# garymm/starflate

Hardware: AMD Instinct MI355X
Metric: compress MiB/s + ratio vs zlib -6, 1 GiB synthetic; 1/2/4/8 GPU (higher is better)
Workload: dtype u8; 1 GPU; 1 GiB synthetic enwik-like text per GPU (gen_text_torch seed 3); effort=default, block_bytes=524288, deflate_block_bytes=32768, window_bytes=32768, container=raw, parallelism=shard1

## Files before the change

### starflate_amd/csrc/sf_kernels.hip

```cpp
#include "sf_device.h"

#include <stdlib.h>

namespace sf {

__device__ __forceinline__ uint32_t len_symbol(uint32_t l3, uint32_t& ebits, uint32_t& eval) {
  if (l3 == 255) { ebits = 0; eval = 0; return 285; }
  if (l3 < 8) { ebits = 0; eval = 0; return 257 + l3; }
  const uint32_t e = (31 - __builtin_clz(l3)) - 2;
  ebits = e;
  eval = l3 & ((1u << e) - 1);
  return 257 + 4 * e + 4 + ((l3 >> e) & 3);
}
__device__ __forceinline__ uint32_t dist_symbol(uint32_t d1, uint32_t& ebits, uint32_t& eval) {
  if (d1 < 4) { ebits = 0; eval = 0; return d1; }
  const uint32_t hb = 31 - __builtin_clz(d1);
  const uint32_t e = hb - 1;
  ebits = e;
  eval = d1 & ((1u << e) - 1);
  return 2 * hb + ((d1 >> e) & 1);
}
__device__ __forceinline__ uint32_t dist_symbol_of(uint32_t d1) {
  const uint32_t x = d1 > 2u ? d1 : 2u;
  const uint32_t hb = 31 - __builtin_clz(x);
// ... 1416 lines not shown
    if (lane < 29) hist[(uint64_t)chunk * kHistStride + 257 + lane] = S.freq[257 + lane];
  }

  stamp();
  if (MODE == 1 && strategy == 0) {
    uint32_t fixb = 0, extra = 0, tot = 0;
    for (uint32_t s0 = lane; s0 < 286; s0 += 64) tot += S.freq[s0];
    tot = wave_sum(tot);
    const uint32_t ltot = est_log2(tot);
    uint32_t ent = 0;
    for (uint32_t s0 = lane; s0 < 286; s0 += 64) {
      const uint32_t f = S.freq[s0];
      if (f) ent += f * (ltot - est_log2(f));
      fixb += f * fixed_ll_len(s0);
      if (s0 >= 257) extra += f * len_extra_of_sym(s0 - 257);
    }
    const uint32_t g = lane < 30 ? S.freq[kHistD + lane] : 0u;
    const uint32_t nmat = wave_sum(g);
    if (g) ent += g * (est_log2(nmat) - est_log2(g));
    if (lane < 30) extra += g * dist_extra_of_sym(lane);
    const uint32_t extra_all = wave_sum(extra);
    const uint32_t est_bits = (wave_sum(ent) >> 8) + extra_all + kEstHeaderBits;
    const uint32_t fixbits = 3 + wave_sum(fixb) + extra_all + 5 * nmat;
    const uint32_t est_b = fin ? (est_bits + 7) / 8 : (est_bits + 3 + 7) / 8 + 4;
    const uint32_t fix_b = fin ? (fixbits + 7) / 8 : (fixbits + 3 + 7) / 8 + 4;
    const uint32_t sto_b = n_raw + kStoredExtra;
    if (fix_b >= sto_b && est_b + kStoreMargin >= sto_b) {
      ChunkCodes& C0 = codes[chunk];
      for (uint32_t s0 = lane; s0 < 320; s0 += 64) C0.lens[s0] = 0;
      if (lane == 0) {
        C0.header[0] = fin ? 1u : 0u;
        ChunkPlan P;
        P.btype = 0;
        P.out_bytes = sto_b;
        P.header_bits = 3;
        P.body_bits = 0;
        plan[chunk] = P;
        T->done = 1;
      }
      return;
    }
  }
  if constexpr (MODE == 1) {
    const uint32_t m_ll = sort_symbols<5>(S, S.freq, 286, S.lens, lane);
    if (m_ll >= 2)
      for (uint32_t k = lane; k < m_ll; k += 64) {
        const uint32_t key = S.key[k];
        T->key_ll[k] = key;
        T->wt_ll[k] = (uint16_t)(key >> 9);
      }
    __syncthreads();
    const uint32_t m_d = sort_symbols<1>(S, S.freq + kHistD, 30, S.lens + 288, lane);
    if (m_d >= 2 && lane < m_d) {
      const uint32_t key = S.key[lane];
      T->key_d[lane] = key;
      T->wt_d[lane] = (uint16_t)(key >> 9);
    }
    if (lane == 0) { T->done = 0; T->m_ll = m_ll; T->m_d = m_d; }
    return;
  } else {
    const uint32_t m_ll = T->m_ll, m_d = T->m_d;
    if (m_ll < 2) {
      sort_symbols<5>(S, S.freq, 286, S.lens, lane);
    } else {
      if (lane < 16) S.cnt[lane] = 0;
      for (uint32_t k = lane; k < m_ll; k += 64) S.key[k] = T->key_ll[k];
      for (uint32_t v = lane; v < 2 * m_ll - 2; v += 64) S.parent[v] = T->parent_ll[v];
      __syncthreads();
      finish_lengths(S, m_ll, 15, S.lens, lane);
    }
    stamp();
    if (m_d < 2) {
      sort_symbols<1>(S, S.freq + kHistD, 30, S.lens + 288, lane);
    } else {
      if (lane < 16) S.cnt[lane] = 0;
      if (lane < m_d) S.key[lane] = T->key_d[lane];
      if (lane < 2 * m_d - 2) S.parent[lane] = T->parent_d[lane];
      __syncthreads();
      finish_lengths(S, m_d, 15, S.lens + 288, lane);
    }
    stamp();
  }

  uint32_t dyn = 0, fix = 0, extra = 0, nmatch = 0;
  for (uint32_t s = lane; s < 286; s += 64) {
    const uint32_t f = S.freq[s];
    dyn += f * S.lens[s];
    fix += f * fixed_ll_len(s);
    if (s >= 257) extra += f * len_extra_of_sym(s - 257);
  }
  if (lane < 30) {
    const uint32_t f = S.freq[kHistD + lane];
    dyn += f * S.lens[288 + lane];
    extra += f * dist_extra_of_sym(lane);
    nmatch += f;
  }
  dyn = wave_sum(dyn);
  fix = wave_sum(fix);
  extra = wave_sum(extra);
  nmatch = wave_sum(nmatch);
  const uint32_t dyn_body = dyn + extra;
  const uint32_t fix_body = fix + extra + 5 * nmatch;

  if (lane < 32) S.clfreq[lane] = 0;
  for (uint32_t k = lane; k < kHeaderWords; k += 64) s_header[k] = 0;
  __syncthreads();
  uint32_t hlit, hdist;
  {
    const uint64_t m4 = __ballot(256 + lane < 286 && S.lens[256 + lane] != 0);
    hlit = 256 + 64 - (uint32_t)__builtin_clzll(m4);
    const uint64_t md = __ballot(lane < 30 && S.lens[288 + lane] != 0);
    hdist = md ? 64 - (uint32_t)__builtin_clzll(md) : 1u;
  }
  const uint32_t nl = rle_parallel(S, S.lens, hlit, 0, lane);
  const uint32_t nd = rle_parallel(S, S.lens + 288, hdist, nl, lane);
  const uint32_t nitems = nl + nd;
  __syncthreads();
  stamp();
  build_lengths(S, S.clfreq, 19, 7, S.cl_lens, lane);
  canonical_codes(S.cl_lens, 19, S.cl_code, lane);
  __syncthreads();
  stamp();
  {
    const uint64_t mc = __ballot(lane < 19 && S.cl_lens[c_cl_order[lane < 19 ? lane : 0]] != 0);
    uint32_t hclen = mc ? 64 - (uint32_t)__builtin_clzll(mc) : 4u;
    hclen = hclen < 4 ? 4u : hclen;
    if (lane == 0)
      or_bits(s_header, 0, (uint64_t)((fin ? 1u : 0u) | (2u << 1) | ((hlit - 257) << 3) | ((hdist - 1) << 8) | ((hclen - 4) << 13)));
    if (lane < hclen) or_bits(s_header, 17 + 3 * lane, (uint64_t)S.cl_lens[c_cl_order[lane]]);
    uint32_t bitbase = 17 + 3 * hclen;
#pragma unroll
    for (uint32_t g = 0; g < 5; ++g) {
      if (g * 64 >= nitems) break;
      const uint32_t k = g * 64 + lane;
      uint32_t nb = 0;
      uint64_t v = 0;
      if (k < nitems) {
        const uint32_t sy = S.rle_sym[k];
        const uint32_t c = S.cl_code[sy];
        const uint32_t cl = c >> 16;
        const uint32_t eb = sy == 16 ? 2u : sy == 17 ? 3u : sy == 18 ? 7u : 0u;
        v = (uint64_t)(c & 0xFFFF) | ((uint64_t)S.rle_ext[k] << cl);
        nb = cl + eb;
      }
      const uint32_t incl = wave_incl_add(nb);
      if (nb) or_bits(s_header, bitbase + incl - nb, v);
      bitbase += (uint32_t)__builtin_amdgcn_readlane((int)incl, 63);
    }
    if (lane == 0) S.cnt[0] = bitbase;
  }
  __syncthreads();

  stamp();
  const uint32_t dyn_hbits = S.cnt[0];
  const uint32_t dyn_bits = dyn_hbits + dyn_body;
  const uint32_t fix_bits = 3 + fix_body;
  const uint32_t dyn_bytes = fin ? (dyn_bits + 7) / 8 : (dyn_bits + 3 + 7) / 8 + 4;
  const uint32_t fix_bytes = fin ? (fix_bits + 7) / 8 : (fix_bits + 3 + 7) / 8 + 4;
  const uint32_t sto_bytes = n_raw + kStoredExtra;
  uint32_t bt;
  if (strategy == 1) bt = 0;
  else if (strategy == 2) bt = 1;
  else if (strategy == 3) bt = 2;
  else {
    bt = 0;
    uint32_t best = sto_bytes;
    if (fix_bytes < best) { bt = 1; best = fix_bytes; }
    if (dyn_bytes < best) { bt = 2; best = dyn_bytes; }
  }

  ChunkCodes& C = codes[chunk];
  for (uint32_t s = lane; s < 320; s += 64) C.lens[s] = S.lens[s];
  __syncthreads();
  if (bt == 1) {
    for (uint32_t s = lane; s < 320; s += 64) S.lens[s] = s < 288 ? (uint8_t)fixed_ll_len(s) : (uint8_t)5;
    if (lane == 0) s_header[0] = (fin ? 1u : 0u) | (1u << 1);
    __syncthreads();
  } else if (bt == 0) {
    if (lane == 0) s_header[0] = fin ? 1u : 0u;
    __syncthreads();
  }
  canonical_codes(S.lens, 288, C.lcode, lane);
  canonical_codes(S.lens + 288, 32, C.dcode, lane);
  const uint32_t hbits = bt == 2 ? dyn_hbits : 3;
  for (uint32_t k = lane; k < (hbits + 31) / 32; k += 64) C.header[k] = s_header[k];
  if (lane == 0) {
    ChunkPlan P;
    P.btype = bt;
    P.out_bytes = bt == 0 ? sto_bytes : bt == 1 ? fix_bytes : dyn_bytes;
    P.header_bits = hbits;
    P.body_bits = bt == 1 ? fix_body : dyn_body;
    plan[chunk] = P;
  }
  stamp();
}

#define SF_PLAN_KERNEL(NAME, MODE)                                                                                          \
  __global__ __launch_bounds__(64) void NAME(uint64_t n_total, uint32_t nchunks, uint32_t* __restrict__ hist,                 \
                                             const uint32_t* __restrict__ ntok, ChunkPlan* __restrict__ plan,                 \
                                             ChunkCodes* __restrict__ codes, uint32_t strategy, uint32_t final_stream,        \
                                             uint64_t* __restrict__ stamps, PlanTree* __restrict__ ptree,                     \
                                             const BatchChunk* __restrict__ bchunks) {                                        \
    plan_chunk<MODE>(n_total, nchunks, hist, ntok, plan, codes, strategy, final_stream, stamps, ptree, bchunks);              \
  }
SF_PLAN_KERNEL(k_plan_sort, 1)
SF_PLAN_KERNEL(k_plan_finish, 2)
#undef SF_PLAN_KERNEL

constexpr uint32_t KM_ROW = 289;
static_assert(2 * KM_ROW >= 576 && (KM_ROW & 1) == 1 && 64 * KM_ROW * 4 <= 80 * 1024, "k_plan_merge: two waves per CU");
__global__ __launch_bounds__(64) void k_plan_merge(uint32_t nchunks, PlanTree* __restrict__ ptree) {
  __shared__ uint32_t s_rows[64 * KM_ROW];
  const uint32_t lane = threadIdx.x;
  const uint32_t chunk = blockIdx.x * 64 + lane;
  if (chunk >= nchunks) return;
  PlanTree* const T = ptree + chunk;
  if (T->done) return;
  uint16_t* const w = reinterpret_cast<uint16_t*>(s_rows + lane * KM_ROW);
  uint32_t* const w32 = s_rows + lane * KM_ROW;
#pragma unroll 1
  for (uint32_t tree = 0; tree < 2; ++tree) {
    const uint32_t m = tree ? T->m_d : T->m_ll;
    if (m < 2) continue;
    const uint32_t* const wt32 = reinterpret_cast<const uint32_t*>(tree ? T->wt_d : T->wt_ll);
    uint16_t* const parent = tree ? T->parent_d : T->parent_ll;
    for (uint32_t k = 0; k < (m + 1) / 2; ++k) w32[k] = wt32[k];
    merge_two_queue_lane(m, [&](uint32_t k) -> uint32_t { return w[k]; }, [&](uint32_t k, uint32_t v) { w[k] = (uint16_t)v; },
                         [&](uint32_t x, uint32_t k) { parent[x] = (uint16_t)k; });
  }
}

constexpr uint32_t K3_THREADS = 1024;
constexpr uint32_t K3_TILES = kBatchChunks / K3_THREADS;
static_assert(kBatchChunks % K3_THREADS == 0 && K3_TILES == 32 && K3_THREADS / 64 == 16, "k_scan: 32 tiles, a DPP row per tile's wave totals");
static_assert((uint64_t)kBatchChunks * (kChunk + kChunk / 8 + 656) < (1ull << 32), "a batch's bytes fit 32 bits");
template <bool BATCH>
__global__ __launch_bounds__(K3_THREADS) void k_scan(uint32_t nchunks, const ChunkPlan* __restrict__ plan,
                                                     uint64_t base, uint32_t carry, uint64_t* __restrict__ offsets,
                                                     uint64_t* __restrict__ total, BatchItem* __restrict__ bitems,
                                                     uint32_t nitems) {
  __shared__ uint32_t s_wt[K3_TILES][16];
  __shared__ uint32_t s_tile[K3_TILES + 1];
  const uint64_t hdr = base;
  if constexpr (BATCH) base = 0;
  else if (carry) base = *total;
  const uint32_t t = threadIdx.x, lane = t & 63, wave = t >> 6;
  uint32_t v[K3_TILES], ex[K3_TILES];
#pragma unroll
  for (uint32_t k = 0; k < K3_TILES; ++k) {
    const uint32_t c = k * K3_THREADS + t;
    v[k] = c < nchunks ? plan[c].out_bytes : 0u;
  }
#pragma unroll
  for (uint32_t k = 0; k < K3_TILES; ++k) {
    const uint32_t incl = wave_incl_add(v[k]);
    ex[k] = incl - v[k];
    if (lane == 63) s_wt[k][wave] = incl;
  }
  __syncthreads();
  if (t < K3_TILES * 16) {
    const uint32_t x = s_wt[t >> 4][t & 15];
    uint32_t r = x;
    r += dpp_from<0x111, 0xF>(r);
    r += dpp_from<0x112, 0xF>(r);
    r += dpp_from<0x114, 0xF>(r);
    r += dpp_from<0x118, 0xF>(r);
    s_wt[t >> 4][t & 15] = r - x;
    if ((t & 15) == 15) s_tile[t >> 4] = r;
  }
  __syncthreads();
  if (wave == 0) {
    const uint32_t x = lane < K3_TILES ? s_tile[lane] : 0u;
    const uint32_t r = wave_incl_add(x);
    if (lane < K3_TILES) s_tile[lane] = r - x;
    if (lane == K3_TILES - 1) s_tile[K3_TILES] = r;
  }
  __syncthreads();
#pragma unroll
  for (uint32_t k = 0; k < K3_TILES; ++k) {
    const uint32_t c = k * K3_THREADS + t;
    if (c < nchunks) offsets[c] = base + s_tile[k] + s_wt[k][wave] + ex[k];
  }
  if (t == 0) {
    const uint64_t all = base + s_tile[K3_TILES];
    if constexpr (!BATCH) *total = all;
    offsets[nchunks] = all;
  }
  if constexpr (BATCH) {
    __syncthreads();
    for (uint32_t i = t; i < nitems; i += K3_THREADS) {
      BatchItem& I = bitems[i];
      const uint64_t g0 = offsets[I.chunk0], g1 = offsets[I.chunk0 + I.nchunks];
      const uint64_t start = I.carry ? total[I.out] : hdr;
      I.shift = start - g0;
      total[I.out] = start + (g1 - g0);
    }
  }
}

constexpr uint32_t K4_THREADS = 512;
constexpr uint32_t K4_WAVES = K4_THREADS / 64;
constexpr uint32_t K4_IPT = 8;
constexpr uint32_t K4_STAGE_FORCED = 9392;
constexpr uint32_t K4_STAGE_AUTO = 8200;
static_assert(4 * K4_STAGE_FORCED >= 3 + kChunk + kChunk / 8 + 640 + 16 + 8, "k_emit: the stage holds the largest chunk");
static_assert(4 * K4_STAGE_AUTO >= 3 + kChunk + kStoredExtra - 1 + 16 + 8, "k_emit: the small stage holds the largest chunk "
              "plan_chunk codes under strategy 0");
static_assert(K4_STAGE_FORCED % 4 == 0 && K4_STAGE_AUTO % 4 == 0, "the stage is zeroed in 16-byte steps");
template <uint32_t STAGE_WORDS>
struct EmitLds {
  alignas(16) uint32_t stage[STAGE_WORDS];
  uint32_t lcode[288];
  uint32_t dcode[32];
  uint32_t tab[1024];
  uint32_t wtot[2][K4_WAVES];
  uint32_t rtok[kSubRegions];
};
template <uint32_t STAGE_WORDS>
constexpr uint32_t k4_waves_per_simd() { return STAGE_WORDS == K4_STAGE_AUTO ? 8 : 6; }
static_assert(k4_waves_per_simd<K4_STAGE_AUTO>() / 2 * sizeof(EmitLds<K4_STAGE_AUTO>) <= 160 * 1024, "k_emit: four workgroups per CU");
static_assert(k4_waves_per_simd<K4_STAGE_FORCED>() / 2 * sizeof(EmitLds<K4_STAGE_FORCED>) <= 160 * 1024, "k_emit: three workgroups per CU");

typedef uint16_t u16x2 __attribute__((ext_vector_type(2)));
typedef int16_t s16x2 __attribute__((ext_vector_type(2)));

__device__ __forceinline__ void literal_bits(uint32_t byte, const uint32_t* lcode, uint64_t& value, uint32_t& nb) {
  const uint32_t lc = lcode[byte];
  value = lc & 0xFFFF;
  nb = lc >> 16;
}
__device__ __forceinline__ uint32_t lenlut_entry(uint32_t l3, const uint32_t* lcode) {
  uint32_t le, lv;
  const uint32_t lc = lcode[len_symbol(l3, le, lv)];
  const uint32_t p = lc >> 16;
  return (lc & 0xFFFFu) | (lv << p) | ((p + le) << 24);
}
__device__ __forceinline__ void match_bits(uint32_t l3, uint32_t d1, const uint32_t* lenlut, const uint32_t* dcode,
                                           uint64_t& value, uint32_t& nb) {
  uint32_t de, dv;
  const uint32_t ds = dist_symbol(d1, de, dv);
  const uint32_t le = lenlut[l3], dc = dcode[ds];
  uint32_t p = le >> 24;
  uint64_t v = le & 0xFFFFFFu;
  v |= (uint64_t)(dc & 0xFFFF) << p;
  p += dc >> 16;
  v |= (uint64_t)dv << p;
  p += de;
  value = v;
  nb = p;
}

template <bool BATCH, uint32_t STAGE_WORDS>
__global__ __launch_bounds__(K4_THREADS, k4_waves_per_simd<STAGE_WORDS>()) void k_emit(const uint8_t* __restrict__ src, uint64_t n_total,
                                                     uint32_t , uint16_t* items,
                                                     const uint32_t* __restrict__ nitems_in,
                                                     const uint32_t* __restrict__ ntok_in,
                                                     const ChunkPlan* __restrict__ plan,
                                                     const ChunkCodes* __restrict__ codes,
                                                     const uint64_t* __restrict__ offsets,
                                                     const uint32_t* __restrict__ rtok,
                                                     uint32_t* __restrict__ subidx,
                                                     uint8_t* __restrict__ dst_all,
                                                     const BatchChunk* __restrict__ bchunks,
                                                     const BatchItem* __restrict__ bitems) {
  __shared__ EmitLds<STAGE_WORDS> L;
  uint32_t(&s_stage)[STAGE_WORDS] = L.stage;
  uint32_t(&s_lcode)[288] = L.lcode;
  uint32_t(&s_dcode)[32] = L.dcode;
  uint32_t(&s_tab)[1024] = L.tab;
  uint32_t(&s_wtot)[2][K4_WAVES] = L.wtot;
  uint32_t(&s_rtok)[kSubRegions] = L.rtok;
  static_assert(K4_THREADS == 512, "one table entry per thread and kind");
  constexpr uint32_t kTabLit = 512, kTabLen = 768, kTabDistN = 510;

  const uint32_t t = threadIdx.x, lane = t & 63;
  const uint32_t wave = (uint32_t)__builtin_amdgcn_readfirstlane((int)(t >> 6));
  const uint32_t chunk = blockIdx.x;
  const ChunkPlan P = plan[chunk];
  const uint8_t* csrc;
  uint8_t* dst;
  uint64_t off = offsets[chunk];
  uint32_t n_raw;
  if constexpr (BATCH) {
    const BatchChunk B = bchunks[chunk];
    const BatchItem& I = bitems[B.item >> 1];
    csrc = B.src;
    n_raw = B.n_raw;
    dst = I.dst;
    off += I.shift;
  } else {
    const uint64_t cbase = (uint64_t)chunk * kChunk;
    csrc = src + cbase;
    n_raw = (uint32_t)((n_total - cbase) < (uint64_t)kChunk ? (n_total - cbase) : kChunk);
    dst = dst_all;
  }
  const ChunkCodes& C = codes[chunk];
  uint32_t pre_code = t < 288 ? C.lcode[t] : (t < 320 ? C.dcode[t - 288] : 0u);
  uint32_t pre_rtok = t < kSubRegions ? rtok[(uint64_t)chunk * kSubRegions + t] : 0u;
  const uint32_t pre_ntok = ntok_in[chunk], pre_nit = nitems_in[chunk];
  asm volatile("" : "+v"(pre_code), "+v"(pre_rtok));

  uint32_t* const sub = subidx + (uint64_t)chunk * 2 * kSubRegions;
  if (P.btype == 0) {
    if (t < 2 * kSubRegions) sub[t] = 0;
    uint8_t* o = dst + off;
    if (t == 0) {
      o[0] = (uint8_t)(C.header[0] & 1u);
      o[1] = (uint8_t)(n_raw & 0xFF);
      o[2] = (uint8_t)(n_raw >> 8);
      o[3] = (uint8_t)(~n_raw & 0xFF);
      o[4] = (uint8_t)((~n_raw >> 8) & 0xFF);
    }
    uint8_t* d = o + 5;
    const uint8_t* sp = csrc;
    if (n_raw >= 64) {
      const uint32_t head16 = (uint32_t)((16 - ((uintptr_t)d & 15)) & 15);
      if (t < head16) d[t] = sp[t];
      const uint32_t sft = head16 & 15u, wsel = sft >> 2, bs = sft & 3u;
      const uint32_t nvec = (n_raw - head16) / 16 - (sft ? 1u : 0u);
      const uint4* s4 = reinterpret_cast<const uint4*>(sp);
      uint4* d4 = reinterpret_cast<uint4*>(d + head16);
      for (uint32_t k = t; k < nvec; k += K4_THREADS) {
        const uint4 A = s4[k + (head16 >> 4)], B = sft ? s4[k + (head16 >> 4) + 1] : make_uint4(0, 0, 0, 0);
        uint4 r;
        if (wsel == 0) {
          r.x = __builtin_amdgcn_alignbyte(A.y, A.x, bs); r.y = __builtin_amdgcn_alignbyte(A.z, A.y, bs);
          r.z = __builtin_amdgcn_alignbyte(A.w, A.z, bs); r.w = __builtin_amdgcn_alignbyte(B.x, A.w, bs);
        } else if (wsel == 1) {
          r.x = __builtin_amdgcn_alignbyte(A.z, A.y, bs); r.y = __builtin_amdgcn_alignbyte(A.w, A.z, bs);
          r.z = __builtin_amdgcn_alignbyte(B.x, A.w, bs); r.w = __builtin_amdgcn_alignbyte(B.y, B.x, bs);
        } else if (wsel == 2) {
          r.x = __builtin_amdgcn_alignbyte(A.w, A.z, bs); r.y = __builtin_amdgcn_alignbyte(B.x, A.w, bs);
          r.z = __builtin_amdgcn_alignbyte(B.y, B.x, bs); r.w = __builtin_amdgcn_alignbyte(B.z, B.y, bs);
        } else {
          r.x = __builtin_amdgcn_alignbyte(B.x, A.w, bs); r.y = __builtin_amdgcn_alignbyte(B.y, B.x, bs);
          r.z = __builtin_amdgcn_alignbyte(B.z, B.y, bs); r.w = __builtin_amdgcn_alignbyte(B.w, B.z, bs);
        }
        d4[k] = r;
      }
      const uint32_t done16 = head16 + 16 * nvec;
      if (t < n_raw - done16) d[done16 + t] = sp[done16 + t];
      return;
    }
    const uint32_t head = (uint32_t)((4 - ((uintptr_t)d & 3)) & 3);
    const uint32_t h = head < n_raw ? head : n_raw;
    if (t < h) d[t] = sp[t];
    const uint32_t nd = (n_raw - h) / 4;
    uint32_t* d32 = reinterpret_cast<uint32_t*>(d + h);
    const uint32_t* s32 = reinterpret_cast<const uint32_t*>(sp);
    const uint32_t full_src_words = n_raw / 4;
    for (uint32_t k = t; k < nd; k += K4_THREADS) {
      const uint32_t ob = h + 4 * k;
      const uint32_t w = ob >> 2;
      uint32_t lo = s32[w], hi = 0;
      if ((ob & 3) != 0) {
        if (w + 1 < full_src_words) hi = s32[w + 1];
        else
          for (uint32_t b = 0; b < 4 && 4 * (w + 1) + b < n_raw; ++b) hi |= (uint32_t)sp[4 * (w + 1) + b] << (8 * b);
      }
      d32[k] = __builtin_amdgcn_alignbyte(hi, lo, ob & 3);
    }
    const uint32_t done = h + 4 * nd;
    if (t < n_raw - done) d[done + t] = sp[done + t];
    return;
  }

  const uint32_t sh = (uint32_t)(off & 3);
  const uint32_t nwords = (sh + P.out_bytes + 3) / 4;
  {
    uint4* z = reinterpret_cast<uint4*>(s_stage);
    for (uint32_t k = t; k < (nwords + 2 + 3) / 4 && k < STAGE_WORDS / 4; k += K4_THREADS) z[k] = make_uint4(0, 0, 0, 0);
  }
  if (t < 288) s_lcode[t] = pre_code;
  else if (t < 320) s_dcode[t - 288] = pre_code;
  if (t < kSubRegions) {
    s_rtok[t] = pre_rtok;
    sub[2 * t + 1] = pre_rtok;
  }
  __syncthreads();
  if (t < 256) {
    const uint32_t le = lenlut_entry(t, s_lcode);
    s_tab[kTabLen + t] = (le & 0xFFFFFu) | (le >> 24) * (1u << 20 | 1u << 27);
    s_tab[kTabLit + t] = (pre_code & 0xFFFFu) | (pre_code >> 16) * (1u << 20 | 1u << 27);
  }
  if (t < kTabDistN) {
    const uint32_t sym = dist_symbol_of(t < 256 ? t : (t - 254) << 7);
    const uint32_t dc = s_dcode[sym];
    s_tab[t] = (dc & 0xFFFFu) | ((dc >> 16) << 20) | (((dc >> 16) + dist_extra_of_sym(sym)) << 27);
  } else {
    s_tab[t] = 0;
  }
  {
    uint8_t* sb = reinterpret_cast<uint8_t*>(s_stage) + sh;
    const uint8_t* hb = reinterpret_cast<const uint8_t*>(C.header);
    const uint32_t hbytes = (P.header_bits + 7) / 8;
    for (uint32_t k = t; k < hbytes; k += K4_THREADS) sb[k] = hb[k];
  }
  __syncthreads();

  const uint32_t ntok = pre_ntok;
  const uint32_t nit = pre_nit & ~kItemsSkipped;
  const uint16_t* it = items + (uint64_t)chunk * kChunk;
  if (pre_nit & kItemsSkipped) {
    uint16_t* const wr = items + (uint64_t)chunk * kChunk;
    for (uint32_t pos = t; pos < nit; pos += K4_THREADS) {
      const uint32_t b = csrc[pos];
      wr[pos] = (uint16_t)(kItemTok | ((pos & (kSubBytes - 1)) == 0 ? (b | kItemRegion | ((pos / kSubBytes) << kItemRegionShift)) : b));
    }
    __threadfence_block();
    __syncthreads();
  }
  uint32_t running = 8 * sh + P.header_bits;
  uint32_t buf = 0;
  uint4 q_next = make_uint4(0, 0, 0, 0);
  if (nit) q_next = *reinterpret_cast<const uint4*>(it + t * K4_IPT);
  for (uint32_t b0 = 0; b0 < nit; b0 += K4_THREADS * K4_IPT, buf ^= 1) {
    const uint32_t i0 = b0 + t * K4_IPT;
    const uint4 q = q_next;
    const bool full = b0 + K4_THREADS * K4_IPT <= nit;
    if (b0 + K4_THREADS * K4_IPT < nit) q_next = *reinterpret_cast<const uint4*>(it + i0 + K4_THREADS * K4_IPT);
    const uint32_t qd[K4_IPT / 2] = {q.x, q.y, q.z, q.w};
    uint32_t val[K4_IPT], nb[K4_IPT], mine = 0;
    uint32_t ent[K4_IPT];
#pragma unroll
    for (uint32_t j = 0; j < K4_IPT / 2; ++j) {
      static_assert(kItemHead == 0x100 && kTabLen == kTabLit + 0x100 && kTabLit == 0x200, "a token's low nine bits are its table index");
      static_assert(kItemTok == 0x8000, "bit 15 tells a token's first item from a distance");
      const u16x2 w = __builtin_bit_cast(u16x2, qd[j]);
      const uint32_t itok = (qd[j] & 0x01FF01FFu) | (kTabLit * 0x10001u);
      const u16x2 idist = __builtin_elementwise_min(w, (u16x2)(w >> (uint16_t)7) + (uint16_t)254);
      uint32_t tok = __builtin_bit_cast(uint32_t, __builtin_bit_cast(s16x2, w) >> (int16_t)15);
      asm volatile("" : "+v"(tok));
      const uint32_t idx = (tok & itok) | (~tok & __builtin_bit_cast(uint32_t, idist));
      const uint32_t by = __builtin_bit_cast(uint32_t, (u16x2)(__builtin_bit_cast(u16x2, idx) << (uint16_t)2));
      ent[2 * j] = *reinterpret_cast<const uint32_t*>(reinterpret_cast<const uint8_t*>(s_tab) + (by & 0xFFFFu));
      ent[2 * j + 1] = *reinterpret_cast<const uint32_t*>(reinterpret_cast<const uint8_t*>(s_tab) + (by >> 16));
    }
    asm volatile("" : "+v"(ent[0]), "+v"(ent[1]), "+v"(ent[2]), "+v"(ent[3]), "+v"(ent[4]), "+v"(ent[5]), "+v"(ent[6]), "+v"(ent[7]));
    auto both = [](uint32_t w) { return w & (w << 1) & 0x80008000u; };
    auto sbit = [](uint32_t k) { return (k & 1) ? 15 + k : k; };
    uint32_t starts = (both(q.x) >> 15) | (both(q.y) >> 13) | (both(q.z) >> 11) | (both(q.w) >> 9);
    if (!full) {
      uint32_t left = nit - i0;
      left = i0 < nit ? left : 0u;
#pragma unroll
      for (uint32_t k = 0; k < K4_IPT; ++k) {
        ent[k] = k < left ? ent[k] : 0u;
        starts &= k < left ? ~0u : ~(1u << sbit(k));
      }
    }
    const uint32_t s0 = starts ? (uint32_t)__builtin_ctz(starts) : 32u;
    const bool walk = __ballot((starts & (starts - 1)) != 0) != 0;
    uint32_t off0 = 0;
#pragma unroll
    for (uint32_t k = 0; k < K4_IPT; ++k) {
      const uint32_t en = ent[k];
      const uint32_t dl = en >> 20, n = en >> 27;
      val[k] = (__builtin_amdgcn_ubfe(qd[k / 2], 16 * (k & 1), (n - dl) & 31u) << (dl & 31u)) | (en & 0xFFFFFu);
      nb[k] = n;
      asm volatile("" : "+v"(val[k]), "+v"(nb[k]));
      off0 = s0 == sbit(k) ? mine : off0;
      mine += nb[k];
    }
    uint32_t region0;
    {
      const uint32_t j = (s0 >> 1) & 3u;
      const uint32_t w = j == 0 ? q.x : j == 1 ? q.y : j == 2 ? q.z : q.w;
      region0 = (w >> ((s0 & 16u) + kItemRegionShift)) & 31u;
    }
    const uint32_t incl = wave_incl_add(mine);
    if (lane == 63) s_wtot[buf][wave] = incl;
    __syncthreads();
    uint32_t pre = 0, all = 0;
#pragma unroll
    for (uint32_t w = 0; w < K4_WAVES; ++w) {
      const uint32_t v = s_wtot[buf][w];
      if (w < wave) pre += v;
      all += v;
    }
    const uint32_t pos = running + pre + incl - mine;
    if (walk) {
      const uint4 r = *reinterpret_cast<const uint4*>(it + i0);
      const uint32_t rd[K4_IPT / 2] = {r.x, r.y, r.z, r.w};
      uint32_t pk = pos;
#pragma unroll
      for (uint32_t k = 0; k < K4_IPT; ++k) {
        const uint32_t e = (rd[k / 2] >> (16 * (k & 1))) & 0xFFFFu;
        if ((e & (kItemTok | kItemRegion)) == (kItemTok | kItemRegion) && i0 + k < nit)
          sub[2 * ((e >> kItemRegionShift) & 31u)] = pk - 8 * sh;
        pk += nb[k];
      }
    } else if (starts) {
      sub[2 * region0] = pos + off0 - 8 * sh;
    }
    uint32_t wi = pos >> 5, ab = pos & 31;
    uint64_t acc = 0;
    auto put = [&](uint32_t v32, uint32_t n) {
      acc |= (uint64_t)v32 << ab;
      ab += n;
      if (ab >= 32) {
        atomicOr(&s_stage[wi++], (uint32_t)acc);
        acc >>= 32;
        ab -= 32;
      }
    };
#pragma unroll
    for (uint32_t k = 0; k < K4_IPT; ++k) put(val[k], nb[k]);
    if (ab) atomicOr(&s_stage[wi], (uint32_t)acc);
    running += all;
  }
  __syncthreads();
  if (t < kSubRegions && s_rtok[t] >= ntok) sub[2 * t] = running - 8 * sh;
  if (t == 0) {
    const uint32_t eob = s_lcode[256];
    or_bits(s_stage, running, eob & 0xFFFF);
    const uint32_t endbit = running + (eob >> 16);
    if (!(C.header[0] & 1u)) {
      const uint32_t byte = (endbit + 3 + 7) / 8;
      or_bits(s_stage, 8 * (byte + 2), 0xFFFFull);
    }
  }
  __syncthreads();

  uint8_t* gbase = dst + (off - sh);
  uint32_t* g32 = reinterpret_cast<uint32_t*>(gbase);
  const uint32_t lo_b = sh, hi_b = sh + P.out_bytes;
  for (uint32_t w = t; w < nwords; w += K4_THREADS) {
    const uint32_t v = s_stage[w];
    if (4 * w >= lo_b && 4 * w + 4 <= hi_b) {
      g32[w] = v;
    } else {
#pragma unroll
      for (uint32_t b = 0; b < 4; ++b) {
        const uint32_t idx = 4 * w + b;
        if (idx >= lo_b && idx < hi_b) gbase[idx] = (uint8_t)(v >> (8 * b));
      }
    }
  }
}

hipError_t init_kernels() { return hipSuccess; }

hipError_t launch_lz77(const uint8_t* src, uint64_t n, uint32_t nchunks, const Workspace& ws,
                       const Options& opt, hipStream_t s, const BatchTables* bt) {
  if (opt.strip_bytes == 0 || opt.strip_bytes % kChunk || opt.strip_bytes > kMaxStrip) return hipErrorInvalidValue;
  if (opt.fast_skip == 2 && opt.strategy != 0) return hipErrorInvalidValue;
  const uint32_t per = opt.strip_bytes / kChunk;
  const uint32_t nstrips = bt ? bt->nstrips : (nchunks + per - 1) / per;
  const BatchStrip* strips = bt ? bt->strips : nullptr;
  const auto launch = [&](auto kernel, uint64_t* stamps) {
    hipLaunchKernelGGL(kernel, dim3(nstrips), dim3(K1_THREADS), 0, s, src, n, opt.strip_bytes, ws.items, ws.nitems, ws.ntok,
                       ws.hist, ws.rtok, opt.lazy, opt.fast_skip, stamps, opt.chain_depth, strips);
  };
#define SF_K1(D2, NR, S2, LG, CH, RC)                                                                                     \
  (ws.stamps && !bt ? launch(k_lz77<true, D2, NR, S2, LG, CH, RC>, ws.stamps)                                          \
   : !bt ? launch(k_lz77<false, D2, NR, S2, LG, CH, RC>, (uint64_t*)nullptr)                                           \
         : launch(k_lz77<false, D2, NR, S2, LG, CH, RC, true>, (uint64_t*)nullptr))
  if (opt.recent) {
    if (opt.stride2) SF_K1(true, true, true, false, false, true);
    else SF_K1(true, true, false, false, false, true);
  } else if (opt.chain_depth) {
    SF_K1(true, true, false, false, true, false);
  } else {
    const uint32_t kind = !opt.stride2 ? (opt.long_table ? 4u : 3u) : opt.depth2 ? 0u : (opt.near ? 1u : 2u);
    if (kind == 0) SF_K1(true, true, true, false, false, false);
    else if (kind == 1) SF_K1(false, true, true, false, false, false);
    else if (kind == 2) SF_K1(false, false, true, false, false, false);
    else if (kind == 3) SF_K1(true, true, false, false, false, false);
    else SF_K1(true, true, false, true, false, false);
  }
#undef SF_K1
  return hipGetLastError();
}
hipError_t launch_plan(uint64_t n, uint32_t nchunks, const Workspace& ws, const Options& opt,
                       hipStream_t s, const BatchTables* bt) {
  const BatchChunk* bchunks = bt ? bt->chunks : nullptr;
  if (!ws.ptree) return hipErrorInvalidValue;
  hipLaunchKernelGGL(k_plan_sort, dim3(nchunks), dim3(64), 0, s, n, nchunks, ws.hist, ws.ntok, ws.plan, ws.codes,
                     opt.strategy, opt.final_stream, (uint64_t*)nullptr, ws.ptree, bchunks);
  hipLaunchKernelGGL(k_plan_merge, dim3((nchunks + 63) / 64), dim3(64), 0, s, nchunks, ws.ptree);
  hipLaunchKernelGGL(k_plan_finish, dim3(nchunks), dim3(64), 0, s, n, nchunks, ws.hist, ws.ntok, ws.plan, ws.codes,
                     opt.strategy, opt.final_stream, ws.stamps, ws.ptree, bchunks);
  return hipGetLastError();
}
hipError_t launch_scan(uint32_t nchunks, const Workspace& ws, uint64_t base, bool carry, uint64_t* d_total, hipStream_t s,
                       const BatchTables* bt) {
  if (nchunks > kBatchChunks) return hipErrorInvalidValue;
  if (bt)
    hipLaunchKernelGGL(k_scan<true>, dim3(1), dim3(K3_THREADS), 0, s, nchunks, ws.plan, base, 0u, ws.offsets, d_total, bt->items,
                       bt->nitems);
  else
    hipLaunchKernelGGL(k_scan<false>, dim3(1), dim3(K3_THREADS), 0, s, nchunks, ws.plan, base, carry ? 1u : 0u, ws.offsets, d_total,
                       (BatchItem*)nullptr, 0u);
  return hipGetLastError();
}
__global__ __launch_bounds__(256) void k_batch_index(const BatchChunk* __restrict__ chunks, const BatchIndexRow* __restrict__ rows,
                                                     const BatchItem* __restrict__ pieces, const uint64_t* __restrict__ offsets,
                                                     const uint64_t* __restrict__ total, uint32_t nchunks, uint64_t* __restrict__ index) {
  const uint32_t c = blockIdx.x * 256 + threadIdx.x;
  if (c >= nchunks) return;
  const BatchIndexRow R = rows[c];
  const uint64_t e = (uint64_t)c + R.item;
  index[e] = offsets[c] + pieces[R.piece].shift;
  if (chunks[c].item & 1u) index[e + 1] = total[R.item];
}
hipError_t launch_batch_index(const BatchChunk* chunks, const BatchIndexRow* rows, const BatchItem* pieces, const uint64_t* offsets,
                              const uint64_t* total, uint32_t nchunks, uint64_t* index, hipStream_t s) {
  hipLaunchKernelGGL(k_batch_index, dim3((nchunks + 255) / 256), dim3(256), 0, s, chunks, rows, pieces, offsets, total, nchunks, index);
  return hipGetLastError();
}
hipError_t launch_emit(const uint8_t* src, uint64_t n, uint32_t nchunks, const Workspace& ws, const Options& opt,
                       uint8_t* dst, hipStream_t s, const BatchTables* bt) {
  const auto launch = [&](auto kernel) {
    hipLaunchKernelGGL(kernel, dim3(nchunks), dim3(K4_THREADS), 0, s, src, n, nchunks, ws.items, ws.nitems, ws.ntok, ws.plan,
                       ws.codes, ws.offsets, ws.rtok, ws.subidx, dst, bt ? bt->chunks : (const BatchChunk*)nullptr,
                       bt ? (const BatchItem*)bt->items : (const BatchItem*)nullptr);
  };
  const bool forced = opt.strategy == 2 || opt.strategy == 3;
  if (bt) forced ? launch(k_emit<true, K4_STAGE_FORCED>) : launch(k_emit<true, K4_STAGE_AUTO>);
  else forced ? launch(k_emit<false, K4_STAGE_FORCED>) : launch(k_emit<false, K4_STAGE_AUTO>);
  return hipGetLastError();
}

}
```

Before: 224,200 MiB/s.

## Align emit staging to 16 bytes for vector stores and skip idle waves

The emit kernel now aligns its LDS bit stage to the 16-byte alignment of the destination pointer instead of 4 bytes. This lets the final flush use uint4 global stores for the interior, with a few byte stores at the edges. Waves whose slice of the final partial batch has no items now skip the table lookups, scan and atomics, writing a zero wave total instead. The stage grows by a few words to cover the larger shift, at a small LDS cost.

```diff
diff --git a/starflate_amd/csrc/sf_kernels.hip b/starflate_amd/csrc/sf_kernels.hip
--- a/starflate_amd/csrc/sf_kernels.hip
+++ b/starflate_amd/csrc/sf_kernels.hip
@@ -1742,11 +1742,11 @@
 constexpr uint32_t K4_WAVES = K4_THREADS / 64;
 constexpr uint32_t K4_IPT = 8;
 constexpr uint32_t K4_STAGE_FORCED = 9392;
-constexpr uint32_t K4_STAGE_AUTO = 8200;
-static_assert(4 * K4_STAGE_FORCED >= 3 + kChunk + kChunk / 8 + 640 + 16 + 8, "k_emit: the stage holds the largest chunk");
-static_assert(4 * K4_STAGE_AUTO >= 3 + kChunk + kStoredExtra - 1 + 16 + 8, "k_emit: the small stage holds the largest chunk "
+constexpr uint32_t K4_STAGE_AUTO = 8204;
+static_assert(4 * K4_STAGE_FORCED >= 15 + kChunk + kChunk / 8 + 640 + 16 + 8, "k_emit: the stage holds the largest chunk");
+static_assert(4 * K4_STAGE_AUTO >= 15 + kChunk + kStoredExtra - 1 + 16 + 8, "k_emit: the small stage holds the largest chunk "
               "plan_chunk codes under strategy 0");
-static_assert(K4_STAGE_FORCED % 4 == 0 && K4_STAGE_AUTO % 4 == 0, "the stage is zeroed in 16-byte steps");
+static_assert(K4_STAGE_FORCED % 4 == 0 && K4_STAGE_AUTO % 4 == 0, "the stage is zeroed, and flushed, in 16-byte steps");
 template <uint32_t STAGE_WORDS>
 struct EmitLds {
   alignas(16) uint32_t stage[STAGE_WORDS];
@@ -1905,7 +1905,7 @@
     return;
   }
 
-  const uint32_t sh = (uint32_t)(off & 3);
+  const uint32_t sh = (uint32_t)(reinterpret_cast<uintptr_t>(dst + off) & 15);
   const uint32_t nwords = (sh + P.out_bytes + 3) / 4;
   {
     uint4* z = reinterpret_cast<uint4*>(s_stage);
@@ -1960,56 +1960,60 @@
     const bool full = b0 + K4_THREADS * K4_IPT <= nit;
     if (b0 + K4_THREADS * K4_IPT < nit) q_next = *reinterpret_cast<const uint4*>(it + i0 + K4_THREADS * K4_IPT);
     const uint32_t qd[K4_IPT / 2] = {q.x, q.y, q.z, q.w};
-    uint32_t val[K4_IPT], nb[K4_IPT], mine = 0;
-    uint32_t ent[K4_IPT];
-#pragma unroll
-    for (uint32_t j = 0; j < K4_IPT / 2; ++j) {
-      static_assert(kItemHead == 0x100 && kTabLen == kTabLit + 0x100 && kTabLit == 0x200, "a token's low nine bits are its table index");
-      static_assert(kItemTok == 0x8000, "bit 15 tells a token's first item from a distance");
-      const u16x2 w = __builtin_bit_cast(u16x2, qd[j]);
-      const uint32_t itok = (qd[j] & 0x01FF01FFu) | (kTabLit * 0x10001u);
-      const u16x2 idist = __builtin_elementwise_min(w, (u16x2)(w >> (uint16_t)7) + (uint16_t)254);
-      uint32_t tok = __builtin_bit_cast(uint32_t, __builtin_bit_cast(s16x2, w) >> (int16_t)15);
-      asm volatile("" : "+v"(tok));
-      const uint32_t idx = (tok & itok) | (~tok & __builtin_bit_cast(uint32_t, idist));
-      const uint32_t by = __builtin_bit_cast(uint32_t, (u16x2)(__builtin_bit_cast(u16x2, idx) << (uint16_t)2));
-      ent[2 * j] = *reinterpret_cast<const uint32_t*>(reinterpret_cast<const uint8_t*>(s_tab) + (by & 0xFFFFu));
-      ent[2 * j + 1] = *reinterpret_cast<const uint32_t*>(reinterpret_cast<const uint8_t*>(s_tab) + (by >> 16));
-    }
-    asm volatile("" : "+v"(ent[0]), "+v"(ent[1]), "+v"(ent[2]), "+v"(ent[3]), "+v"(ent[4]), "+v"(ent[5]), "+v"(ent[6]), "+v"(ent[7]));
-    auto both = [](uint32_t w) { return w & (w << 1) & 0x80008000u; };
-    auto sbit = [](uint32_t k) { return (k & 1) ? 15 + k : k; };
-    uint32_t starts = (both(q.x) >> 15) | (both(q.y) >> 13) | (both(q.z) >> 11) | (both(q.w) >> 9);
-    if (!full) {
-      uint32_t left = nit - i0;
-      left = i0 < nit ? left : 0u;
+    const bool idle = b0 + wave * (64 * K4_IPT) >= nit;
+    uint32_t val[K4_IPT], nb[K4_IPT], mine = 0, incl = 0, starts = 0, s0 = 32u, off0 = 0, region0 = 0;
+    bool walk = false;
+    if (!idle) {
+      uint32_t ent[K4_IPT];
+#pragma unroll
+      for (uint32_t j = 0; j < K4_IPT / 2; ++j) {
+        static_assert(kItemHead == 0x100 && kTabLen == kTabLit + 0x100 && kTabLit == 0x200, "a token's low nine bits are its table index");
+        static_assert(kItemTok == 0x8000, "bit 15 tells a token's first item from a distance");
+        const u16x2 w = __builtin_bit_cast(u16x2, qd[j]);
+        const uint32_t itok = (qd[j] & 0x01FF01FFu) | (kTabLit * 0x10001u);
+        const u16x2 idist = __builtin_elementwise_min(w, (u16x2)(w >> (uint16_t)7) + (uint16_t)254);
+        uint32_t tok = __builtin_bit_cast(uint32_t, __builtin_bit_cast(s16x2, w) >> (int16_t)15);
+        asm volatile("" : "+v"(tok));
+        const uint32_t idx = (tok & itok) | (~tok & __builtin_bit_cast(uint32_t, idist));
+        const uint32_t by = __builtin_bit_cast(uint32_t, (u16x2)(__builtin_bit_cast(u16x2, idx) << (uint16_t)2));
+        ent[2 * j] = *reinterpret_cast<const uint32_t*>(reinterpret_cast<const uint8_t*>(s_tab) + (by & 0xFFFFu));
+        ent[2 * j + 1] = *reinterpret_cast<const uint32_t*>(reinterpret_cast<const uint8_t*>(s_tab) + (by >> 16));
+      }
+      asm volatile("" : "+v"(ent[0]), "+v"(ent[1]), "+v"(ent[2]), "+v"(ent[3]), "+v"(ent[4]), "+v"(ent[5]), "+v"(ent[6]), "+v"(ent[7]));
+      auto both = [](uint32_t w) { return w & (w << 1) & 0x80008000u; };
+      auto sbit = [](uint32_t k) { return (k & 1) ? 15 + k : k; };
+      starts = (both(q.x) >> 15) | (both(q.y) >> 13) | (both(q.z) >> 11) | (both(q.w) >> 9);
+      if (!full) {
+        uint32_t left = nit - i0;
+        left = i0 < nit ? left : 0u;
+#pragma unroll
+        for (uint32_t k = 0; k < K4_IPT; ++k) {
+          ent[k] = k < left ? ent[k] : 0u;
+          starts &= k < left ? ~0u : ~(1u << sbit(k));
+        }
+      }
+      s0 = starts ? (uint32_t)__builtin_ctz(starts) : 32u;
+      walk = __ballot((starts & (starts - 1)) != 0) != 0;
 #pragma unroll
       for (uint32_t k = 0; k < K4_IPT; ++k) {
-        ent[k] = k < left ? ent[k] : 0u;
-        starts &= k < left ? ~0u : ~(1u << sbit(k));
-      }
-    }
-    const uint32_t s0 = starts ? (uint32_t)__builtin_ctz(starts) : 32u;
-    const bool walk = __ballot((starts & (starts - 1)) != 0) != 0;
-    uint32_t off0 = 0;
-#pragma unroll
-    for (uint32_t k = 0; k < K4_IPT; ++k) {
-      const uint32_t en = ent[k];
-      const uint32_t dl = en >> 20, n = en >> 27;
-      val[k] = (__builtin_amdgcn_ubfe(qd[k / 2], 16 * (k & 1), (n - dl) & 31u) << (dl & 31u)) | (en & 0xFFFFFu);
-      nb[k] = n;
-      asm volatile("" : "+v"(val[k]), "+v"(nb[k]));
-      off0 = s0 == sbit(k) ? mine : off0;
-      mine += nb[k];
-    }
-    uint32_t region0;
-    {
-      const uint32_t j = (s0 >> 1) & 3u;
-      const uint32_t w = j == 0 ? q.x : j == 1 ? q.y : j == 2 ? q.z : q.w;
-      region0 = (w >> ((s0 & 16u) + kItemRegionShift)) & 31u;
-    }
-    const uint32_t incl = wave_incl_add(mine);
-    if (lane == 63) s_wtot[buf][wave] = incl;
+        const uint32_t en = ent[k];
+        const uint32_t dl = en >> 20, n = en >> 27;
+        val[k] = (__builtin_amdgcn_ubfe(qd[k / 2], 16 * (k & 1), (n - dl) & 31u) << (dl & 31u)) | (en & 0xFFFFFu);
+        nb[k] = n;
+        asm volatile("" : "+v"(val[k]), "+v"(nb[k]));
+        off0 = s0 == sbit(k) ? mine : off0;
+        mine += nb[k];
+      }
+      {
+        const uint32_t j = (s0 >> 1) & 3u;
+        const uint32_t w = j == 0 ? q.x : j == 1 ? q.y : j == 2 ? q.z : q.w;
+        region0 = (w >> ((s0 & 16u) + kItemRegionShift)) & 31u;
+      }
+      incl = wave_incl_add(mine);
+      if (lane == 63) s_wtot[buf][wave] = incl;
+    } else if (lane == 63) {
+      s_wtot[buf][wave] = 0;
+    }
     __syncthreads();
     uint32_t pre = 0, all = 0;
 #pragma unroll
@@ -2018,35 +2022,37 @@
       if (w < wave) pre += v;
       all += v;
     }
-    const uint32_t pos = running + pre + incl - mine;
-    if (walk) {
-      const uint4 r = *reinterpret_cast<const uint4*>(it + i0);
-      const uint32_t rd[K4_IPT / 2] = {r.x, r.y, r.z, r.w};
-      uint32_t pk = pos;
-#pragma unroll
-      for (uint32_t k = 0; k < K4_IPT; ++k) {
-        const uint32_t e = (rd[k / 2] >> (16 * (k & 1))) & 0xFFFFu;
-        if ((e & (kItemTok | kItemRegion)) == (kItemTok | kItemRegion) && i0 + k < nit)
-          sub[2 * ((e >> kItemRegionShift) & 31u)] = pk - 8 * sh;
-        pk += nb[k];
-      }
-    } else if (starts) {
-      sub[2 * region0] = pos + off0 - 8 * sh;
-    }
-    uint32_t wi = pos >> 5, ab = pos & 31;
-    uint64_t acc = 0;
-    auto put = [&](uint32_t v32, uint32_t n) {
-      acc |= (uint64_t)v32 << ab;
-      ab += n;
-      if (ab >= 32) {
-        atomicOr(&s_stage[wi++], (uint32_t)acc);
-        acc >>= 32;
-        ab -= 32;
-      }
-    };
-#pragma unroll
-    for (uint32_t k = 0; k < K4_IPT; ++k) put(val[k], nb[k]);
-    if (ab) atomicOr(&s_stage[wi], (uint32_t)acc);
+    if (!idle) {
+      const uint32_t pos = running + pre + incl - mine;
+      if (walk) {
+        const uint4 r = *reinterpret_cast<const uint4*>(it + i0);
+        const uint32_t rd[K4_IPT / 2] = {r.x, r.y, r.z, r.w};
+        uint32_t pk = pos;
+#pragma unroll
+        for (uint32_t k = 0; k < K4_IPT; ++k) {
+          const uint32_t e = (rd[k / 2] >> (16 * (k & 1))) & 0xFFFFu;
+          if ((e & (kItemTok | kItemRegion)) == (kItemTok | kItemRegion) && i0 + k < nit)
+            sub[2 * ((e >> kItemRegionShift) & 31u)] = pk - 8 * sh;
+          pk += nb[k];
+        }
+      } else if (starts) {
+        sub[2 * region0] = pos + off0 - 8 * sh;
+      }
+      uint32_t wi = pos >> 5, ab = pos & 31;
+      uint64_t acc = 0;
+      auto put = [&](uint32_t v32, uint32_t n) {
+        acc |= (uint64_t)v32 << ab;
+        ab += n;
+        if (ab >= 32) {
+          atomicOr(&s_stage[wi++], (uint32_t)acc);
+          acc >>= 32;
+          ab -= 32;
+        }
+      };
+#pragma unroll
+      for (uint32_t k = 0; k < K4_IPT; ++k) put(val[k], nb[k]);
+      if (ab) atomicOr(&s_stage[wi], (uint32_t)acc);
+    }
     running += all;
   }
   __syncthreads();
@@ -2063,19 +2069,19 @@
   __syncthreads();
 
   uint8_t* gbase = dst + (off - sh);
-  uint32_t* g32 = reinterpret_cast<uint32_t*>(gbase);
   const uint32_t lo_b = sh, hi_b = sh + P.out_bytes;
-  for (uint32_t w = t; w < nwords; w += K4_THREADS) {
-    const uint32_t v = s_stage[w];
-    if (4 * w >= lo_b && 4 * w + 4 <= hi_b) {
-      g32[w] = v;
-    } else {
-#pragma unroll
-      for (uint32_t b = 0; b < 4; ++b) {
-        const uint32_t idx = 4 * w + b;
-        if (idx >= lo_b && idx < hi_b) gbase[idx] = (uint8_t)(v >> (8 * b));
-      }
-    }
+  const uint32_t kb0 = (lo_b + 15) / 16, kb1 = hi_b / 16;
+  {
+    const uint4* s4 = reinterpret_cast<const uint4*>(s_stage);
+    uint4* g4 = reinterpret_cast<uint4*>(gbase);
+    for (uint32_t k = kb0 + t; k < kb1; k += K4_THREADS) g4[k] = s4[k];
+  }
+  const uint8_t* sbytes = reinterpret_cast<const uint8_t*>(s_stage);
+  if (t < 16) {
+    if (t >= lo_b && t < hi_b && t < 16 * kb0) gbase[t] = sbytes[t];
+  } else if (t >= 64 && t < 80) {
+    const uint32_t idx = 16 * kb1 + (t - 64);
+    if (idx >= 16 * kb0 && idx < hi_b) gbase[idx] = sbytes[idx];
   }
 }
 
```

New measurement: 226,100 MiB/s (median of 6 runs). Within noise of the previous version (+0.8%).
